# Tony-Tseng/deep-rawburst-sr

Hardware: AMD Instinct MI355X
Metric: bursts/sec 14x48x48 RAW->4x (SyntheticBurstVal shape), DBSR forward (higher is better)
Workload: dtype fp16; 1 GPU; configs[1]: SyntheticBurstVal 14-frame 48x48 -> 384x384 (sr x8 of RAW, x4 of full-res), batch 8 per GPU, full PWC-Net + warp + fusion + decoder; global_batch=8, frames=14, height=48, width=48, out_size=384, parallelism=dp1 (independent bursts per rank), hip_graph=True, fusion_weights_written=True

## Files before the change

### deep-rawburst-sr_amd/csrc/conv128.hip

```cpp
#include "conv_core.hpp"

#include <algorithm>

namespace dbsr {

namespace ks128 {
constexpr int HW = TW + 2, HH = TH + 2, HPX = HW * HH;
constexpr int CPX = 184;
constexpr int NCH = 4;
constexpr int CH_U4 = CPX * 4;
constexpr int PIECES = NCH * CPX / 16;
constexpr int BUF_U4 = NCH * CH_U4;
constexpr int NW = 8;
constexpr int PER = (PIECES + NW - 1) / NW;
#ifndef DBSR_KS_NB
#define DBSR_KS_NB 2
#endif
#ifndef DBSR_KS_ABL
#define DBSR_KS_ABL 0
#endif
#ifndef DBSR_KS_RING
#define DBSR_KS_RING 3
#endif
constexpr int NB = DBSR_KS_NB;
constexpr int RING = DBSR_KS_RING;
constexpr int HALF = TH / 2;
constexpr int XCH_U4 = NW * HALF * 2 * 64;
constexpr int LDS_U4 = 2 * BUF_U4 + XCH_U4;
static_assert(LDS_U4 * 16 + 128 * 4 <= 160 * 1024, "ks128 LDS");
static_assert(CPX % 8 == 0 && CPX >= HPX && (NCH * CPX) % 16 == 0, "chunk images");
static_assert(HALF % NB == 0, "batches");
}

template <typename T, int EPI>
__global__ __launch_bounds__(512, 1) void conv3x3_ks128_kernel(ConvK k, int tiles_x, int tiles_y, int ntiles) {
    using namespace ks128;
    DBSR_OWN_SIMDS();
    __shared__ __attribute__((aligned(16))) u32x4_t lds[LDS_U4 + 32];
    u32x4_t* xch = lds + 2 * BUF_U4;
    float* lbias = (float*)(lds + LDS_U4);
    const int lane = threadIdx.x & 63, wave = __builtin_amdgcn_readfirstlane(threadIdx.x >> 6);
    const int kh = wave >> 2, q = wave & 3;
    const int H = k.in_h, W = k.in_w;
    constexpr bool RT = EPI == 0 || EPI == 5, has_gate = EPI == 5;
    const bool has_res = EPI == 2 || (RT && k.r != nullptr);
    auto act1 = [&](float v) {
        if constexpr (EPI == 1) return fmaxf(v, 0.f);
        else if constexpr (RT) return apply_act(v, k.act);
        else return v;
    };
    auto act2 = [&](float v) {
        if constexpr (EPI == 2) return fmaxf(v, 0.f);
        else if constexpr (RT) return apply_act(v, k.post_act);
        else return v;
    };

    Frag<T> w[2][9][2];
    {
        const char* wsrc = (const char*)k.w_pipe;
#pragma unroll
        for (int c = 0; c < 2; ++c)
#pragma unroll
            for (int tap = 0; tap < 9; ++tap)
#pragma unroll
                for (int h = 0; h < 2; ++h)
                    w[c][tap][h].load((const T*)(wsrc + (((2 * q + h) * NCH + 2 * kh + c) * 9 + tap) * 1024 + lane * 16));
    }
    if (threadIdx.x < 128) lbias[threadIdx.x] = k.bias ? k.bias[threadIdx.x] : 0.f;
    struct Tile { const T* xf; long long y_off, r_off, g_off; int y0, x0; };
    auto decode = [&](int i) {
        const int t = rb_tile(i, blockIdx.x, gridDim.x, ntiles);
        const int tx = t % tiles_x, r = t / tiles_x, ty = r % tiles_y, f = r / tiles_y;
        Tile tl;
        tl.y0 = ty * TH; tl.x0 = tx * TW;
        tl.xf = (const T*)k.x + map_frame(k.xm, f) * k.x_is;
        const long long pix = (long long)tl.y0 * k.out_w + tl.x0;
        tl.y_off = map_frame(k.ym, f) * k.y_is + k.y_c0 + pix * k.y_ld;
        tl.r_off = has_res ? map_frame(k.rm, f) * k.r_is + k.r_c0 + pix * k.r_ld : 0;
        tl.g_off = has_gate ? map_frame(k.gm, f) * k.g_is + k.g_c0 + pix * k.g_ld : 0;
        return tl;
    };
    const int my_tiles = ntiles / (int)gridDim.x + ((int)blockIdx.x < ntiles % (int)gridDim.x ? 1 : 0);

    const int pix_b = k.x_ld * (int)sizeof(T);
    const unsigned frame_bytes = (unsigned)((long long)H * W * pix_b);
    const unsigned lds0 = (unsigned)(unsigned long long)(__attribute__((address_space(3))) u32x4_t*)lds;
    int h_rc[PER], h_off[PER];
#pragma unroll
    for (int it = 0; it < PER; ++it) {
        const int item = min(wave + NW * it, PIECES - 1);
        const int qq = item * 16 + (lane >> 2), c = qq / CPX, p = qq - c * CPX, ph = lane & 3;
        const int gg = 2 * ((ph & 1) ^ ((p >> 2) & 1)) + (ph >> 1);
        const int r = p / HW, cc = p - r * HW;
        h_rc[it] = p < HPX ? (r << 16) | cc : 0x7fff7fff;
        h_off[it] = (r * W + cc) * pix_b + c * 64 + gg * 16;
    }
    auto dma = [&](int it, const Tile& tl, int buf) {
        const int item = min(wave + NW * it, PIECES - 1);
        const int hy = tl.y0 - 1 + (h_rc[it] >> 16), hx = tl.x0 - 1 + (h_rc[it] & 0xffff);
        const bool ok = (unsigned)hy < (unsigned)H && (unsigned)hx < (unsigned)W;
        const int base = ((tl.y0 - 1) * W + (tl.x0 - 1)) * pix_b;
        lds_dma16(tl.xf, frame_bytes, ok ? base + h_off[it] : BUF_OOB, 0,
                  lds0 + (unsigned)((buf * BUF_U4 + item * 64) * 16));
    };

    auto taps = [&](int buf, auto j0_, f32x4_t (&acc)[NB][2], auto&& hook) {
        constexpr int J0 = decltype(j0_)::value, NS = 18;
        if constexpr ((DBSR_KS_ABL & 1) != 0) {
            for (int j = 0; j < NB; ++j) acc[j][0] = acc[j][1] = f32x4_t{(float)(J0 + j + buf), 0.f, 0.f, 0.f};
            StaticFor<0, NS>::run([&](auto s_) { hook(decltype(s_)::value); });
            return;
        }
        const int g = lane >> 4, col = lane & 15;
        const unsigned base = lds0 + (unsigned)((buf * BUF_U4 + kh * 2 * CH_U4) * 16);
        unsigned ba[8];
#pragma unroll
        for (int rho = 0; rho < 8; ++rho) ba[rho] = base + 16u * (4 * col + halo_phys(col + rho, g));
        Frag<T> bq[NB][RING];
        constexpr int AH = RING - 1;
        auto rd = [&](auto j_, auto st_) {
            constexpr int j = decltype(j_)::value, st = decltype(st_)::value;
            constexpr int c = st / 9, tap = st % 9, imm = (J0 + j + tap / 3) * HW + tap % 3;
            const unsigned a = ba[imm & 7];
            bf16x8_t v;
            asm volatile("ds_read_b128 %0, %1 offset:%2" : "=v"(v) : "v"(a), "i"(16 * (c * CH_U4 + 4 * imm)));
            bq[j][st % RING].v = v;
        };
        StaticFor<0, AH>::run([&](auto s0_) {
            StaticFor<0, NB>::run([&](auto j_) { rd(j_, s0_); });
        });
        StaticFor<0, NS>::run([&](auto s_) {
            constexpr int st = decltype(s_)::value, c = st / 9, tap = st % 9;
            const f32x4_t z = {0.f, 0.f, 0.f, 0.f};
            StaticFor<0, NB>::run([&](auto j_) {
                constexpr int j = decltype(j_)::value;
                constexpr int mid = (AH - 1 < NS - 1 - st) ? AH - 1 : NS - 1 - st;
                constexpr int newer = (NB - 1 - j) + NB * mid + (st + AH < NS ? j : 0);
                bf16x8_t v = bq[j][st % RING].v;
                asm volatile("s_waitcnt lgkmcnt(%1)" : "+v"(v) : "i"(newer));
                bq[j][st % RING].v = v;
                acc[j][0] = mma(w[c][tap][0], bq[j][st % RING], st == 0 ? z : acc[j][0]);
                acc[j][1] = mma(w[c][tap][1], bq[j][st % RING], st == 0 ? z : acc[j][1]);
                if constexpr (st + AH < NS) rd(j_, std::integral_constant<int, st + AH>{});
            });
            hook(st);
        });
    };

    Tile cur = decode(0);
    if (my_tiles > 0) {
#pragma unroll
        for (int it = 0; it < PER; ++it) dma(it, cur, 0);
    }
    const int own0 = HALF * kh;
    for (int ti = 0; ti < my_tiles; ++ti) {
        if (ti == 0) vm_drain();
        else DBSR_VM_WAIT(HALF);
        __syncthreads();
        const bool more = ti + 1 < my_tiles;
        const Tile nxt = more ? decode(ti + 1) : cur;
        const int buf = ti & 1;
        int ln = lane;
        asm volatile("" : "+v"(ln));
        const int g = ln >> 4, col = ln & 15;
        StaticFor<0, HALF / NB>::run([&](auto b_) {
            constexpr int b = decltype(b_)::value;
            f32x4_t acc[NB][2];
            auto hook = [&](int st) {
                if constexpr (b == 0 && (DBSR_KS_ABL & 2) == 0) {
                    if (more) {
#pragma unroll
                        for (int it = 0; it < PER; ++it)
                            if (st == 2 * it + 1) dma(it, nxt, buf ^ 1);
                    }
                }
            };
            if (kh == 0) taps(buf, std::integral_constant<int, HALF + NB * b>{}, acc, hook);
            else taps(buf, std::integral_constant<int, NB * b>{}, acc, hook);
#pragma unroll
            for (int j = 0; j < NB; ++j)
#pragma unroll
                for (int h = 0; h < 2; ++h)
                    if constexpr ((DBSR_KS_ABL & 4) == 0)
                        xch[((wave * HALF + NB * b + j) * 2 + h) * 64 + ln] = __builtin_bit_cast(u32x4_t, acc[j][h]);
                    else if (acc[j][h][0] == 12345.f) xch[ln] = u32x4_t{0u, 0u, 0u, 0u};
        });
        u32x4_t resv[HALF];
        auto load_res = [&]() {
#pragma unroll
            for (int j = 0; j < HALF; ++j)
                resv[j] = *(const u32x4_t*)((const T*)k.r + cur.r_off + ((long long)(own0 + j) * k.out_w + col) * k.r_ld +
                                            32 * q + 8 * g);
        };
        if (!RT && has_res) load_res();
        f32x4_t mine[HALF][2];
        StaticFor<0, HALF / NB>::run([&](auto b_) {
            constexpr int b = decltype(b_)::value;
            f32x4_t acc[NB][2];
            auto hook = [&](int) {};
            if (kh == 0) taps(buf, std::integral_constant<int, NB * b>{}, acc, hook);
            else taps(buf, std::integral_constant<int, HALF + NB * b>{}, acc, hook);
#pragma unroll
            for (int j = 0; j < NB; ++j) {
                mine[NB * b + j][0] = acc[j][0];
                mine[NB * b + j][1] = acc[j][1];
            }
        });
        if constexpr ((DBSR_KS_ABL & 4) == 0) dma_barrier();
        const int partner = wave ^ 4;
        const float4 b0 = *(const float4*)(lbias + 32 * q + 8 * g), b1 = *(const float4*)(lbias + 32 * q + 8 * g + 4);
        const float bv[8] = {b0.x, b0.y, b0.z, b0.w, b1.x, b1.y, b1.z, b1.w};
        if (RT && has_res) load_res();
        u32x4_t gatev[has_gate ? HALF : 1];
        if constexpr (has_gate) {
#pragma unroll
            for (int j = 0; j < HALF; ++j)
                gatev[j] = *(const u32x4_t*)((const T*)k.gt + cur.g_off + ((long long)(own0 + j) * k.out_w + col) * k.g_ld +
                                             32 * q + 8 * g);
        }
#pragma unroll
        for (int j = 0; j < HALF; ++j) {
            f32x4_t o0 = {0.f, 0.f, 0.f, 0.f}, o1 = o0;
            if constexpr ((DBSR_KS_ABL & 4) == 0) {
                o0 = __builtin_bit_cast(f32x4_t, xch[((partner * HALF + j) * 2 + 0) * 64 + ln]);
                o1 = __builtin_bit_cast(f32x4_t, xch[((partner * HALF + j) * 2 + 1) * 64 + ln]);
            }
            float v[8];
#pragma unroll
            for (int r = 0; r < 4; ++r) {
                v[r] = act1((mine[j][0][r] + o0[r]) + bv[r]);
                v[4 + r] = act1((mine[j][1][r] + o1[r]) + bv[4 + r]);
            }
            if (has_res) {
#pragma unroll
                for (int e = 0; e < 4; ++e) {
                    v[2 * e] = act2(v[2 * e] + H16<T>::lo(resv[j][e]));
                    v[2 * e + 1] = act2(v[2 * e + 1] + H16<T>::hi(resv[j][e]));
                }
            }
            if constexpr (has_gate) {
#pragma unroll
                for (int e = 0; e < 4; ++e) {
                    v[2 * e] = H16<T>::lo(gatev[j][e]) > 0.f ? v[2 * e] : 0.f;
                    v[2 * e + 1] = H16<T>::hi(gatev[j][e]) > 0.f ? v[2 * e + 1] : 0.f;
                }
            }
            u32x4_t o;
#pragma unroll
            for (int e = 0; e < 4; ++e) o[e] = H16<T>::pack(v[2 * e], v[2 * e + 1]);
            *(u32x4_t*)((T*)k.y + cur.y_off + ((long long)(own0 + j) * k.out_w + col) * k.y_ld + 32 * q + 8 * g) = o;
        }
        cur = nxt;
    }
    vm_drain();
}

int ks128_launch(const ConvK& k, int n_frames, bool f16, int epi, int max_blocks, int cus, hipStream_t s) {
    const int tiles_x = k.out_w / ks128::TW, tiles_y = k.out_h / ks128::TH;
    const long long nt = (long long)n_frames * tiles_x * tiles_y;
    DBSR_CHECK_ARG(nt > 0 && nt < (1LL << 31), "conv2d: bad tile count for the K-split 128-channel kernel");
    const int ntiles = (int)nt;
    int grid = max_blocks > 0 ? std::min(max_blocks, cus) : cus;
    grid = std::min(grid, ntiles);
    DBSR_CHECK_ARG(rb_mapping_ok(grid, ntiles), "conv2d: tile mapping out of range (grid %d, %d tiles)", grid, ntiles);
#define DBSR_KS_LAUNCH(TT, E) \
    hipLaunchKernelGGL((conv3x3_ks128_kernel<TT, E>), dim3(grid), dim3(512), 0, s, k, tiles_x, tiles_y, ntiles)
#define DBSR_KS_EPI(TT)                          \
    switch (epi) {                               \
        case 1: DBSR_KS_LAUNCH(TT, 1); break;    \
        case 2: DBSR_KS_LAUNCH(TT, 2); break;    \
        case 3: DBSR_KS_LAUNCH(TT, 3); break;    \
        case 5: DBSR_KS_LAUNCH(TT, 5); break;    \
        default: DBSR_KS_LAUNCH(TT, 0); break;   \
    }
    if (f16) {
        DBSR_KS_EPI(f16_t)
    } else {
        DBSR_KS_EPI(bf16_t)
    }
#undef DBSR_KS_EPI
#undef DBSR_KS_LAUNCH
    DBSR_LAUNCH_CHECK();
    return 0;
}

}
```

### deep-rawburst-sr_amd/csrc/conv_core.hpp

```cpp
#pragma once
#include "common.hpp"

#include <vector>

namespace dbsr {

inline int round_up(int a, int b) { return (a + b - 1) / b * b; }
inline int cin_pad(int cin) { return cin <= 16 ? round_up(cin, 8) : round_up(cin, 32); }


inline bool is16(int dtype) { return dtype == DBSR_BF16 || dtype == DBSR_F16; }
inline int esize(int dtype) { return is16(dtype) ? 2 : 4; }


struct ConvK {
    const void* x; long long x_is; int x_ld; dbsr_frame_map xm; int in_h, in_w;
    const void* w; const float* bias; int Kp, KG, KGp, CG, kw, stride, pad, dil, cout;
    void* y; int y_f32; long long y_is; int y_ld, y_c0; dbsr_frame_map ym; int out_h, out_w;
    int act;
    const void* r; long long r_is; int r_ld, r_c0; dbsr_frame_map rm; int post_act;
    const void* gt; long long g_is; int g_ld, g_c0; dbsr_frame_map gm;
    int out_mode, shuffle, cps;
    int npix;
    int vec_store;
    int ksplit;
    float* ws;
    int cw;
    const void* w_pipe;
    int max_blocks;
    const float* head_w;
    const float* head_b;
    int head_cout;
    int stage_epi;
};

template <typename T> struct Frag;
template <> struct Frag<bf16_t> {
    bf16x8_t v;
    __device__ __forceinline__ void load(const bf16_t* p) { v = *(const bf16x8_t*)p; }
    __device__ __forceinline__ void zero() { v = bf16x8_t{0, 0, 0, 0, 0, 0, 0, 0}; }
};
template <> struct Frag<f16_t> {
    bf16x8_t v;
    __device__ __forceinline__ void load(const f16_t* p) { v = *(const bf16x8_t*)p; }
    __device__ __forceinline__ void zero() { v = bf16x8_t{0, 0, 0, 0, 0, 0, 0, 0}; }
};
template <> struct Frag<float> {
    float4 a, b;
    __device__ __forceinline__ void load(const float* p) { a = *(const float4*)p; b = *(const float4*)(p + 4); }
    __device__ __forceinline__ void load(const bf16_t* p) {
        const u32x4_t q = *(const u32x4_t*)p;
        a = make_float4(__uint_as_float(q[0] << 16), __uint_as_float(q[0] & 0xffff0000u),
                        __uint_as_float(q[1] << 16), __uint_as_float(q[1] & 0xffff0000u));
        b = make_float4(__uint_as_float(q[2] << 16), __uint_as_float(q[2] & 0xffff0000u),
                        __uint_as_float(q[3] << 16), __uint_as_float(q[3] & 0xffff0000u));
    }
    __device__ __forceinline__ void load(const f16_t* p) {
        const u32x4_t q = *(const u32x4_t*)p;
        a = make_float4(H16<f16_t>::lo(q[0]), H16<f16_t>::hi(q[0]), H16<f16_t>::lo(q[1]), H16<f16_t>::hi(q[1]));
        b = make_float4(H16<f16_t>::lo(q[2]), H16<f16_t>::hi(q[2]), H16<f16_t>::lo(q[3]), H16<f16_t>::hi(q[3]));
    }
    __device__ __forceinline__ void zero() { a = make_float4(0, 0, 0, 0); b = a; }
};

__device__ __forceinline__ f32x4_t mma(const Frag<bf16_t>& A, const Frag<bf16_t>& B, f32x4_t c) {
    typedef __attribute__((ext_vector_type(8))) __bf16 bfv;
    return __builtin_amdgcn_mfma_f32_16x16x32_bf16(__builtin_bit_cast(bfv, A.v), __builtin_bit_cast(bfv, B.v), c,
                                                   0, 0, 0);
}
__device__ __forceinline__ f32x4_t mma(const Frag<f16_t>& A, const Frag<f16_t>& B, f32x4_t c) {
    typedef __attribute__((ext_vector_type(8))) _Float16 hv;
    return __builtin_amdgcn_mfma_f32_16x16x32_f16(__builtin_bit_cast(hv, A.v), __builtin_bit_cast(hv, B.v), c, 0, 0, 0);
}
__device__ __forceinline__ f32x4_t mma(const Frag<float>& A, const Frag<float>& B, f32x4_t c) {
    c = __builtin_amdgcn_mfma_f32_16x16x4f32(A.a.x, B.a.x, c, 0, 0, 0);
    c = __builtin_amdgcn_mfma_f32_16x16x4f32(A.a.y, B.a.y, c, 0, 0, 0);
    c = __builtin_amdgcn_mfma_f32_16x16x4f32(A.a.z, B.a.z, c, 0, 0, 0);
    c = __builtin_amdgcn_mfma_f32_16x16x4f32(A.a.w, B.a.w, c, 0, 0, 0);
    c = __builtin_amdgcn_mfma_f32_16x16x4f32(A.b.x, B.b.x, c, 0, 0, 0);
    c = __builtin_amdgcn_mfma_f32_16x16x4f32(A.b.y, B.b.y, c, 0, 0, 0);
    c = __builtin_amdgcn_mfma_f32_16x16x4f32(A.b.z, B.b.z, c, 0, 0, 0);
    c = __builtin_amdgcn_mfma_f32_16x16x4f32(A.b.w, B.b.w, c, 0, 0, 0);
    return c;
}


__device__ __forceinline__ unsigned relu16x2(unsigned v) {
    typedef short s16x2 __attribute__((ext_vector_type(2)));
    return __builtin_bit_cast(unsigned, __builtin_elementwise_max(__builtin_bit_cast(s16x2, v), s16x2{0, 0}));
}
__device__ __forceinline__ int halo_phys(int p, int g) { return 2 * (g & 1) + ((g >> 1) ^ ((p >> 2) & 1)); }


__host__ __device__ __forceinline__ int rb_tile(int i, int b, int nb, int ntiles) {
    if (nb == 256 && (i + 1) * 256 <= ntiles) return i * 256 + (b & 7) * 32 + (b >> 3);
    return i * nb + b;
}


inline bool rb_mapping_ok(int nb, int ntiles) {
    std::vector<unsigned char> seen(ntiles, 0);
    for (int b = 0; b < nb; ++b) {
        const int my = ntiles / nb + (b < ntiles % nb ? 1 : 0);
        for (int i = 0; i < my; ++i) {
            const int t = rb_tile(i, b, nb, ntiles);
            if (t < 0 || t >= ntiles || seen[t]) return false;
            seen[t] = 1;
        }
    }
    return true;
}

int resblock64_launch(const ConvK& k1, const ConvK& k2, int n_frames, bool f16, int max_blocks, int cus,
                      hipStream_t s);
namespace rb64 {
constexpr int TW = 16, TH = 8;
}

int ks128_launch(const ConvK& k, int n_frames, bool f16, int epi, int max_blocks, int cus, hipStream_t s);
namespace ks128 {
constexpr int TW = 16, TH = 8;
}

}
```

Measured before the change: 3271 bursts/s.

## Rewrite 128-channel conv as weight-stationary row-rolling kernel without K-split exchange

Replaces the K-split scheme, where two wave groups each handle half the input chunks and swap partial sums through LDS, with a weight-stationary design. Each wave now owns 16 output channels across all 4 input chunks and keeps those weights in registers. The taps are rolled over halo rows so each LDS read feeds up to three row accumulators, and the epilogue combines output-row pairs with permlane32_swap. This removes the LDS exchange buffer, the extra barrier and the duplicated halo reads, and interleaves the next-tile DMA and residual/gate loads into the MFMA stream on a compile-time checked schedule. The cost is higher register pressure from 36 weight fragments and 8 accumulators per wave, plus a new host-side validation of launch arguments.

```diff
diff --git a/deep-rawburst-sr_amd/csrc/conv128.hip b/deep-rawburst-sr_amd/csrc/conv128.hip
--- a/deep-rawburst-sr_amd/csrc/conv128.hip
+++ b/deep-rawburst-sr_amd/csrc/conv128.hip
@@ -3,44 +3,14 @@
 #include <algorithm>
 
 namespace dbsr {
-
-namespace ks128 {
-constexpr int HW = TW + 2, HH = TH + 2, HPX = HW * HH;
-constexpr int CPX = 184;
-constexpr int NCH = 4;
-constexpr int CH_U4 = CPX * 4;
-constexpr int PIECES = NCH * CPX / 16;
-constexpr int BUF_U4 = NCH * CH_U4;
-constexpr int NW = 8;
-constexpr int PER = (PIECES + NW - 1) / NW;
-#ifndef DBSR_KS_NB
-#define DBSR_KS_NB 2
-#endif
-#ifndef DBSR_KS_ABL
-#define DBSR_KS_ABL 0
-#endif
-#ifndef DBSR_KS_RING
-#define DBSR_KS_RING 3
-#endif
-constexpr int NB = DBSR_KS_NB;
-constexpr int RING = DBSR_KS_RING;
-constexpr int HALF = TH / 2;
-constexpr int XCH_U4 = NW * HALF * 2 * 64;
-constexpr int LDS_U4 = 2 * BUF_U4 + XCH_U4;
-static_assert(LDS_U4 * 16 + 128 * 4 <= 160 * 1024, "ks128 LDS");
-static_assert(CPX % 8 == 0 && CPX >= HPX && (NCH * CPX) % 16 == 0, "chunk images");
-static_assert(HALF % NB == 0, "batches");
-}
 
 template <typename T, int EPI>
 __global__ __launch_bounds__(512, 1) void conv3x3_ks128_kernel(ConvK k, int tiles_x, int tiles_y, int ntiles) {
     using namespace ks128;
     DBSR_OWN_SIMDS();
-    __shared__ __attribute__((aligned(16))) u32x4_t lds[LDS_U4 + 32];
-    u32x4_t* xch = lds + 2 * BUF_U4;
-    float* lbias = (float*)(lds + LDS_U4);
+    __shared__ __attribute__((aligned(16))) u32x4_t lds[LDS_U4];
     const int lane = threadIdx.x & 63, wave = __builtin_amdgcn_readfirstlane(threadIdx.x >> 6);
-    const int kh = wave >> 2, q = wave & 3;
+    const int g = lane >> 4, col = lane & 15;
     const int H = k.in_h, W = k.in_w;
     constexpr bool RT = EPI == 0 || EPI == 5, has_gate = EPI == 5;
     const bool has_res = EPI == 2 || (RT && k.r != nullptr);
@@ -55,18 +25,23 @@
         else return v;
     };
 
-    Frag<T> w[2][9][2];
+    Frag<T> w[NCH][9];
     {
-        const char* wsrc = (const char*)k.w_pipe;
-#pragma unroll
-        for (int c = 0; c < 2; ++c)
-#pragma unroll
-            for (int tap = 0; tap < 9; ++tap)
-#pragma unroll
-                for (int h = 0; h < 2; ++h)
-                    w[c][tap][h].load((const T*)(wsrc + (((2 * q + h) * NCH + 2 * kh + c) * 9 + tap) * 1024 + lane * 16));
-    }
-    if (threadIdx.x < 128) lbias[threadIdx.x] = k.bias ? k.bias[threadIdx.x] : 0.f;
+        const int m = col;
+        const char* wsrc = (const char*)k.w_pipe + (size_t)packed_block(wave, m) * (NCH * 9 * 1024) +
+                           (g * 16 + packed_row(wave, m)) * 16;
+#pragma unroll
+        for (int c = 0; c < NCH; ++c)
+#pragma unroll
+            for (int tap = 0; tap < 9; ++tap) w[c][tap].load((const T*)(wsrc + (c * 9 + tap) * 1024));
+    }
+    const int co4 = lane_cout(wave, 4 * g), co8 = 16 * wave + 8 * (g & 1);
+    float bv[4];
+#pragma unroll
+    for (int r = 0; r < 4; ++r) bv[r] = k.bias ? k.bias[co4 + r] : 0.f;
+    const int prow = (g >> 1) * k.out_w + col;
+    const int yl = prow * k.y_ld + co8, rl = has_res ? prow * k.r_ld + co8 : 0, gl = has_gate ? prow * k.g_ld + co8 : 0;
+
     struct Tile { const T* xf; long long y_off, r_off, g_off; int y0, x0; };
     auto decode = [&](int i) {
         const int t = rb_tile(i, blockIdx.x, gridDim.x, ntiles);
@@ -85,180 +60,141 @@
     const int pix_b = k.x_ld * (int)sizeof(T);
     const unsigned frame_bytes = (unsigned)((long long)H * W * pix_b);
     const unsigned lds0 = (unsigned)(unsigned long long)(__attribute__((address_space(3))) u32x4_t*)lds;
-    int h_rc[PER], h_off[PER];
-#pragma unroll
-    for (int it = 0; it < PER; ++it) {
+    auto piece = [&](int it, int ln, int& rc, int& off) {
         const int item = min(wave + NW * it, PIECES - 1);
-        const int qq = item * 16 + (lane >> 2), c = qq / CPX, p = qq - c * CPX, ph = lane & 3;
-        const int gg = 2 * ((ph & 1) ^ ((p >> 2) & 1)) + (ph >> 1);
+        const int qq = item * 16 + (ln >> 2), c = qq / CPX, p = qq - c * CPX, ph = ln & 3;
+        const int gg = piece_kgroup(p, ph);
         const int r = p / HW, cc = p - r * HW;
-        h_rc[it] = p < HPX ? (r << 16) | cc : 0x7fff7fff;
-        h_off[it] = (r * W + cc) * pix_b + c * 64 + gg * 16;
+        rc = p < HPX ? (r << 16) | cc : 0x7fff7fff;
+        off = (r * W + cc) * pix_b + c * 64 + gg * 16;
+    };
+    int h_rc[RT ? 1 : PER], h_off[RT ? 1 : PER];
+    if constexpr (!RT) {
+#pragma unroll
+        for (int it = 0; it < PER; ++it) piece(it, lane, h_rc[it], h_off[it]);
     }
     auto dma = [&](int it, const Tile& tl, int buf) {
         const int item = min(wave + NW * it, PIECES - 1);
-        const int hy = tl.y0 - 1 + (h_rc[it] >> 16), hx = tl.x0 - 1 + (h_rc[it] & 0xffff);
+        int rc, off;
+        if constexpr (RT) {
+            int ln = lane;
+            asm volatile("" : "+v"(ln));
+            piece(it, ln, rc, off);
+        } else {
+            rc = h_rc[it];
+            off = h_off[it];
+        }
+        const int hy = tl.y0 - 1 + (rc >> 16), hx = tl.x0 - 1 + (rc & 0xffff);
         const bool ok = (unsigned)hy < (unsigned)H && (unsigned)hx < (unsigned)W;
         const int base = ((tl.y0 - 1) * W + (tl.x0 - 1)) * pix_b;
-        lds_dma16(tl.xf, frame_bytes, ok ? base + h_off[it] : BUF_OOB, 0,
-                  lds0 + (unsigned)((buf * BUF_U4 + item * 64) * 16));
-    };
-
-    auto taps = [&](int buf, auto j0_, f32x4_t (&acc)[NB][2], auto&& hook) {
-        constexpr int J0 = decltype(j0_)::value, NS = 18;
-        if constexpr ((DBSR_KS_ABL & 1) != 0) {
-            for (int j = 0; j < NB; ++j) acc[j][0] = acc[j][1] = f32x4_t{(float)(J0 + j + buf), 0.f, 0.f, 0.f};
-            StaticFor<0, NS>::run([&](auto s_) { hook(decltype(s_)::value); });
-            return;
-        }
-        const int g = lane >> 4, col = lane & 15;
-        const unsigned base = lds0 + (unsigned)((buf * BUF_U4 + kh * 2 * CH_U4) * 16);
-        unsigned ba[8];
-#pragma unroll
-        for (int rho = 0; rho < 8; ++rho) ba[rho] = base + 16u * (4 * col + halo_phys(col + rho, g));
-        Frag<T> bq[NB][RING];
-        constexpr int AH = RING - 1;
-        auto rd = [&](auto j_, auto st_) {
-            constexpr int j = decltype(j_)::value, st = decltype(st_)::value;
-            constexpr int c = st / 9, tap = st % 9, imm = (J0 + j + tap / 3) * HW + tap % 3;
-            const unsigned a = ba[imm & 7];
-            bf16x8_t v;
-            asm volatile("ds_read_b128 %0, %1 offset:%2" : "=v"(v) : "v"(a), "i"(16 * (c * CH_U4 + 4 * imm)));
-            bq[j][st % RING].v = v;
-        };
-        StaticFor<0, AH>::run([&](auto s0_) {
-            StaticFor<0, NB>::run([&](auto j_) { rd(j_, s0_); });
-        });
-        StaticFor<0, NS>::run([&](auto s_) {
-            constexpr int st = decltype(s_)::value, c = st / 9, tap = st % 9;
-            const f32x4_t z = {0.f, 0.f, 0.f, 0.f};
-            StaticFor<0, NB>::run([&](auto j_) {
-                constexpr int j = decltype(j_)::value;
-                constexpr int mid = (AH - 1 < NS - 1 - st) ? AH - 1 : NS - 1 - st;
-                constexpr int newer = (NB - 1 - j) + NB * mid + (st + AH < NS ? j : 0);
-                bf16x8_t v = bq[j][st % RING].v;
-                asm volatile("s_waitcnt lgkmcnt(%1)" : "+v"(v) : "i"(newer));
-                bq[j][st % RING].v = v;
-                acc[j][0] = mma(w[c][tap][0], bq[j][st % RING], st == 0 ? z : acc[j][0]);
-                acc[j][1] = mma(w[c][tap][1], bq[j][st % RING], st == 0 ? z : acc[j][1]);
-                if constexpr (st + AH < NS) rd(j_, std::integral_constant<int, st + AH>{});
-            });
-            hook(st);
-        });
-    };
+        lds_dma16(tl.xf, frame_bytes, ok ? base + off : BUF_OOB, 0, lds0 + (unsigned)((buf * BUF_U4 + item * 64) * 16));
+    };
+    unsigned ba[8];
+#pragma unroll
+    for (int rho = 0; rho < 8; ++rho) ba[rho] = lds0 + 16u * (4 * col + frag_slot(col + rho, g));
 
     Tile cur = decode(0);
     if (my_tiles > 0) {
 #pragma unroll
         for (int it = 0; it < PER; ++it) dma(it, cur, 0);
     }
-    const int own0 = HALF * kh;
+    vm_drain();
+    const long long y_pair = 2LL * k.out_w * k.y_ld, r_pair = 2LL * k.out_w * k.r_ld, g_pair = 2LL * k.out_w * k.g_ld;
     for (int ti = 0; ti < my_tiles; ++ti) {
-        if (ti == 0) vm_drain();
-        else DBSR_VM_WAIT(HALF);
+        DBSR_VM_WAIT(TH / 2);
         __syncthreads();
         const bool more = ti + 1 < my_tiles;
         const Tile nxt = more ? decode(ti + 1) : cur;
         const int buf = ti & 1;
-        int ln = lane;
-        asm volatile("" : "+v"(ln));
-        const int g = ln >> 4, col = ln & 15;
-        StaticFor<0, HALF / NB>::run([&](auto b_) {
-            constexpr int b = decltype(b_)::value;
-            f32x4_t acc[NB][2];
-            auto hook = [&](int st) {
-                if constexpr (b == 0 && (DBSR_KS_ABL & 2) == 0) {
-                    if (more) {
-#pragma unroll
-                        for (int it = 0; it < PER; ++it)
-                            if (st == 2 * it + 1) dma(it, nxt, buf ^ 1);
-                    }
-                }
-            };
-            if (kh == 0) taps(buf, std::integral_constant<int, HALF + NB * b>{}, acc, hook);
-            else taps(buf, std::integral_constant<int, NB * b>{}, acc, hook);
-#pragma unroll
-            for (int j = 0; j < NB; ++j)
-#pragma unroll
-                for (int h = 0; h < 2; ++h)
-                    if constexpr ((DBSR_KS_ABL & 4) == 0)
-                        xch[((wave * HALF + NB * b + j) * 2 + h) * 64 + ln] = __builtin_bit_cast(u32x4_t, acc[j][h]);
-                    else if (acc[j][h][0] == 12345.f) xch[ln] = u32x4_t{0u, 0u, 0u, 0u};
-        });
-        u32x4_t resv[HALF];
-        auto load_res = [&]() {
-#pragma unroll
-            for (int j = 0; j < HALF; ++j)
-                resv[j] = *(const u32x4_t*)((const T*)k.r + cur.r_off + ((long long)(own0 + j) * k.out_w + col) * k.r_ld +
-                                            32 * q + 8 * g);
+        f32x4_t acc[TH];
+        u32x4_t resv[TH / 2], gatev[has_gate ? TH / 2 : 1];
+        Frag<T> bq[AHEAD];
+        auto rd = [&](auto n_) {
+            constexpr int n = decltype(n_)::value, c = read_chunk(n), imm = read_pix(n);
+            const unsigned a = ba[imm & 7];
+            bf16x8_t v;
+            asm volatile("ds_read_b128 %0, %1 offset:%2" : "=v"(v) : "v"(a), "i"(16 * (c * CH_U4 + 4 * imm)));
+            bq[n % AHEAD].v = v;
         };
-        if (!RT && has_res) load_res();
-        f32x4_t mine[HALF][2];
-        StaticFor<0, HALF / NB>::run([&](auto b_) {
-            constexpr int b = decltype(b_)::value;
-            f32x4_t acc[NB][2];
-            auto hook = [&](int) {};
-            if (kh == 0) taps(buf, std::integral_constant<int, NB * b>{}, acc, hook);
-            else taps(buf, std::integral_constant<int, HALF + NB * b>{}, acc, hook);
-#pragma unroll
-            for (int j = 0; j < NB; ++j) {
-                mine[NB * b + j][0] = acc[j][0];
-                mine[NB * b + j][1] = acc[j][1];
-            }
-        });
-        if constexpr ((DBSR_KS_ABL & 4) == 0) dma_barrier();
-        const int partner = wave ^ 4;
-        const float4 b0 = *(const float4*)(lbias + 32 * q + 8 * g), b1 = *(const float4*)(lbias + 32 * q + 8 * g + 4);
-        const float bv[8] = {b0.x, b0.y, b0.z, b0.w, b1.x, b1.y, b1.z, b1.w};
-        if (RT && has_res) load_res();
-        u32x4_t gatev[has_gate ? HALF : 1];
-        if constexpr (has_gate) {
-#pragma unroll
-            for (int j = 0; j < HALF; ++j)
-                gatev[j] = *(const u32x4_t*)((const T*)k.gt + cur.g_off + ((long long)(own0 + j) * k.out_w + col) * k.g_ld +
-                                             32 * q + 8 * g);
-        }
-#pragma unroll
-        for (int j = 0; j < HALF; ++j) {
-            f32x4_t o0 = {0.f, 0.f, 0.f, 0.f}, o1 = o0;
-            if constexpr ((DBSR_KS_ABL & 4) == 0) {
-                o0 = __builtin_bit_cast(f32x4_t, xch[((partner * HALF + j) * 2 + 0) * 64 + ln]);
-                o1 = __builtin_bit_cast(f32x4_t, xch[((partner * HALF + j) * 2 + 1) * 64 + ln]);
-            }
+        auto epilogue = [&](auto pr_) {
+            constexpr int pr = decltype(pr_)::value;
+            if (has_res) asm volatile("" : "+v"(resv[pr]));
+            if constexpr (has_gate) asm volatile("" : "+v"(gatev[pr]));
             float v[8];
 #pragma unroll
             for (int r = 0; r < 4; ++r) {
-                v[r] = act1((mine[j][0][r] + o0[r]) + bv[r]);
-                v[4 + r] = act1((mine[j][1][r] + o1[r]) + bv[4 + r]);
+                const float a0 = act1(acc[2 * pr][r] + bv[r]), a1 = act1(acc[2 * pr + 1][r] + bv[r]);
+                const auto s = __builtin_amdgcn_permlane32_swap(__float_as_uint(a0), __float_as_uint(a1), false, false);
+                v[r] = __uint_as_float(s[0]);
+                v[4 + r] = __uint_as_float(s[1]);
             }
             if (has_res) {
 #pragma unroll
                 for (int e = 0; e < 4; ++e) {
-                    v[2 * e] = act2(v[2 * e] + H16<T>::lo(resv[j][e]));
-                    v[2 * e + 1] = act2(v[2 * e + 1] + H16<T>::hi(resv[j][e]));
+                    v[2 * e] = act2(v[2 * e] + H16<T>::lo(resv[pr][e]));
+                    v[2 * e + 1] = act2(v[2 * e + 1] + H16<T>::hi(resv[pr][e]));
                 }
             }
             if constexpr (has_gate) {
 #pragma unroll
                 for (int e = 0; e < 4; ++e) {
-                    v[2 * e] = H16<T>::lo(gatev[j][e]) > 0.f ? v[2 * e] : 0.f;
-                    v[2 * e + 1] = H16<T>::hi(gatev[j][e]) > 0.f ? v[2 * e + 1] : 0.f;
+                    v[2 * e] = H16<T>::lo(gatev[pr][e]) > 0.f ? v[2 * e] : 0.f;
+                    v[2 * e + 1] = H16<T>::hi(gatev[pr][e]) > 0.f ? v[2 * e + 1] : 0.f;
                 }
             }
             u32x4_t o;
 #pragma unroll
             for (int e = 0; e < 4; ++e) o[e] = H16<T>::pack(v[2 * e], v[2 * e + 1]);
-            *(u32x4_t*)((T*)k.y + cur.y_off + ((long long)(own0 + j) * k.out_w + col) * k.y_ld + 32 * q + 8 * g) = o;
-        }
+            *(u32x4_t*)((T*)k.y + cur.y_off + pr * y_pair + yl) = o;
+        };
+
+        StaticFor<0, AHEAD>::run([&](auto n_) { rd(n_); });
+        StaticFor<0, READS>::run([&](auto n_) {
+            constexpr int n = decltype(n_)::value, c = read_chunk(n);
+            constexpr int newer = AHEAD - 1 < READS - 1 - n ? AHEAD - 1 : READS - 1 - n;
+            bf16x8_t v = bq[n % AHEAD].v;
+            asm volatile("s_waitcnt lgkmcnt(%1)" : "+v"(v) : "i"(newer));
+            Frag<T> b;
+            b.v = v;
+            StaticFor<0, 3>::run([&](auto ky_) {
+                constexpr int ky = decltype(ky_)::value;
+                if constexpr (feeds(n, ky)) {
+                    constexpr int y = read_row(n) - ky, tap = 3 * ky + read_kx(n);
+                    const f32x4_t z = {0.f, 0.f, 0.f, 0.f};
+                    acc[y] = mma(w[c][tap], b, kstep(n, ky) == 0 ? z : acc[y]);
+                }
+            });
+            if constexpr (n + AHEAD < READS) rd(std::integral_constant<int, n + AHEAD>{});
+            StaticFor<0, PER>::run([&](auto it_) {
+                constexpr int it = decltype(it_)::value;
+                if constexpr (n == dma_at(it)) {
+                    if (more) dma(it, nxt, buf ^ 1);
+                }
+            });
+            StaticFor<0, TH / 2>::run([&](auto pr_) {
+                constexpr int pr = decltype(pr_)::value;
+                if constexpr (n == res_at(pr, RT)) {
+                    if (has_res) resv[pr] = *(const u32x4_t*)((const T*)k.r + cur.r_off + pr * r_pair + rl);
+                }
+                if constexpr (has_gate && n == gate_at(pr))
+                    gatev[pr] = *(const u32x4_t*)((const T*)k.gt + cur.g_off + pr * g_pair + gl);
+                if constexpr (n == pair_done(pr)) epilogue(pr_);
+            });
+        });
         cur = nxt;
+#pragma unroll
+        for (int rho = 0; rho < 8; ++rho) ba[rho] += buf ? (unsigned)(-BUF_U4 * 16) : (unsigned)(BUF_U4 * 16);
     }
     vm_drain();
 }
 
 int ks128_launch(const ConvK& k, int n_frames, bool f16, int epi, int max_blocks, int cus, hipStream_t s) {
+    const char* why = ks128::launch_error(k.out_h, k.out_w, k.in_h, k.in_w, n_frames, (long long)k.x_ld * 2, k.y_ld,
+                                          k.y_c0, k.r != nullptr, k.r_ld, k.r_c0, k.gt != nullptr, k.g_ld, k.g_c0);
+    DBSR_CHECK_ARG(why == nullptr, "conv2d: the 128-channel weight-stationary kernel cannot run this: %s", why);
     const int tiles_x = k.out_w / ks128::TW, tiles_y = k.out_h / ks128::TH;
     const long long nt = (long long)n_frames * tiles_x * tiles_y;
-    DBSR_CHECK_ARG(nt > 0 && nt < (1LL << 31), "conv2d: bad tile count for the K-split 128-channel kernel");
+    DBSR_CHECK_ARG(nt > 0 && nt < (1LL << 31), "conv2d: bad tile count for the 128-channel weight-stationary kernel");
     const int ntiles = (int)nt;
     int grid = max_blocks > 0 ? std::min(max_blocks, cus) : cus;
     grid = std::min(grid, ntiles);
diff --git a/deep-rawburst-sr_amd/csrc/conv_core.hpp b/deep-rawburst-sr_amd/csrc/conv_core.hpp
--- a/deep-rawburst-sr_amd/csrc/conv_core.hpp
+++ b/deep-rawburst-sr_amd/csrc/conv_core.hpp
@@ -1,5 +1,6 @@
 #pragma once
 #include "common.hpp"
+#include "ks128_sched.hpp"
 
 #include <vector>
 
@@ -118,8 +119,5 @@
 }
 
 int ks128_launch(const ConvK& k, int n_frames, bool f16, int epi, int max_blocks, int cus, hipStream_t s);
-namespace ks128 {
-constexpr int TW = 16, TH = 8;
-}
 
 }
diff --git a/deep-rawburst-sr_amd/csrc/ks128_sched.hpp b/deep-rawburst-sr_amd/csrc/ks128_sched.hpp
--- /dev/null
+++ b/deep-rawburst-sr_amd/csrc/ks128_sched.hpp
@@ -0,0 +1,117 @@
+#pragma once
+
+namespace dbsr {
+namespace ks128 {
+
+constexpr int TW = 16, TH = 8;
+constexpr int HW = TW + 2, HH = TH + 2, HPX = HW * HH;
+constexpr int CPX = 184;
+constexpr int NCH = 4;
+constexpr int CH_U4 = CPX * 4;
+constexpr int PIECES = NCH * CPX / 16;
+constexpr int BUF_U4 = NCH * CH_U4;
+constexpr int NBUF = 2;
+constexpr int NW = 8;
+constexpr int PER = (PIECES + NW - 1) / NW;
+constexpr int LDS_U4 = NBUF * BUF_U4;
+static_assert(LDS_U4 * 16 <= 160 * 1024, "ks128 LDS");
+static_assert(CPX % 8 == 0 && CPX >= HPX && (NCH * CPX) % 16 == 0, "chunk images");
+
+constexpr int frag_slot(int p, int g) { return 2 * (g & 1) + ((g >> 1) ^ ((p >> 2) & 1)); }
+constexpr int piece_kgroup(int p, int ph) { return 2 * ((ph & 1) ^ ((p >> 2) & 1)) + (ph >> 1); }
+constexpr bool swizzle_ok() {
+    for (int p = 0; p < CPX; ++p)
+        for (int g = 0; g < 4; ++g)
+            if (frag_slot(p, g) < 0 || frag_slot(p, g) > 3 || piece_kgroup(p, frag_slot(p, g)) != g) return false;
+    return true;
+}
+static_assert(swizzle_ok(), "ks128 halo swizzle");
+
+constexpr int RPC = HH * 3;
+constexpr int READS = NCH * RPC;
+constexpr int MFMAS = NCH * 9 * TH;
+constexpr int AHEAD = 4;
+constexpr int read_chunk(int n) { return n / RPC; }
+constexpr int read_row(int n) { return n % RPC / 3; }
+constexpr int read_kx(int n) { return n % 3; }
+constexpr int read_pix(int n) { return read_row(n) * HW + read_kx(n); }
+constexpr bool feeds(int n, int ky) { return read_row(n) - ky >= 0 && read_row(n) - ky < TH; }
+constexpr int kstep(int n, int ky) { return read_chunk(n) * 9 + 3 * ky + read_kx(n); }
+constexpr int pair_done(int pr) { return (NCH - 1) * RPC + (2 * pr + 3) * 3 + 2; }
+constexpr int dma_at(int it) { return 3 + 9 * it; }
+constexpr int res_at(int pr, bool late) { return late ? pair_done(pr) - 12 : 2 * RPC + 2 * pr; }
+constexpr int gate_at(int pr) { return pair_done(pr) - 11; }
+
+constexpr bool schedule_ok() {
+    int next[TH] = {}, total = 0;
+    for (int n = 0; n < READS; ++n) {
+        if (read_pix(n) + TW - 1 >= HPX) return false;
+        for (int ky = 0; ky < 3; ++ky)
+            if (feeds(n, ky)) {
+                const int y = read_row(n) - ky;
+                if (kstep(n, ky) != next[y]) return false;
+                ++next[y];
+                ++total;
+            }
+    }
+    for (int y = 0; y < TH; ++y)
+        if (next[y] != NCH * 9) return false;
+    if (total != MFMAS) return false;
+    for (int pr = 0; pr < TH / 2; ++pr) {
+        if (pair_done(pr) >= READS || (pr > 0 && pair_done(pr) <= pair_done(pr - 1))) return false;
+        for (int y = 2 * pr; y < 2 * pr + 2; ++y)
+            for (int n = pair_done(pr) + 1; n < READS; ++n)
+                for (int ky = 0; ky < 3; ++ky)
+                    if (feeds(n, ky) && read_row(n) - ky == y) return false;
+        for (int late = 0; late < 2; ++late)
+            if (res_at(pr, late != 0) < 0 || res_at(pr, late != 0) >= pair_done(pr)) return false;
+        if (gate_at(pr) < 0 || gate_at(pr) >= pair_done(pr)) return false;
+    }
+    for (int it = 0; it < PER; ++it) {
+        if (dma_at(it) < 0 || dma_at(it) >= pair_done(0) || (it > 0 && dma_at(it) <= dma_at(it - 1))) return false;
+        for (int late = 0; late < 2; ++late)
+            if (dma_at(it) >= res_at(0, late != 0)) return false;
+    }
+    return pair_done(TH / 2 - 1) == READS - 1 && AHEAD >= 1 && AHEAD < RPC;
+}
+static_assert(schedule_ok(), "ks128 row-rolling schedule");
+
+constexpr int lane_cout(int p, int m) { return 16 * p + 8 * ((m >> 2) & 1) + 4 * (m >> 3) + (m & 3); }
+constexpr int packed_block(int p, int m) { return 2 * (p >> 1) + (m >> 3); }
+constexpr int packed_row(int p, int m) { return 4 * (2 * (p & 1) + ((m >> 2) & 1)) + (m & 3); }
+constexpr int packed_cout(int blk, int row) {
+    return 64 * (blk >> 2) + 32 * ((blk & 3) >> 1) + 8 * (row >> 2) + 4 * (blk & 1) + (row & 3);
+}
+constexpr bool gather_ok() {
+    bool seen[128] = {};
+    for (int p = 0; p < NW; ++p)
+        for (int m = 0; m < 16; ++m) {
+            const int co = lane_cout(p, m);
+            if (co < 0 || co >= 128 || seen[co]) return false;
+            seen[co] = true;
+            if (packed_block(p, m) < 0 || packed_block(p, m) >= 8 || packed_row(p, m) < 0 || packed_row(p, m) >= 16)
+                return false;
+            if (packed_cout(packed_block(p, m), packed_row(p, m)) != co) return false;
+        }
+    return true;
+}
+static_assert(gather_ok(), "ks128 cout gather");
+
+inline const char* launch_error(int out_h, int out_w, int in_h, int in_w, long long n_frames, long long x_ld_bytes,
+                                int y_ld, int y_c0, bool has_res, int r_ld, int r_c0, bool has_gate, int g_ld,
+                                int g_c0) {
+    if (out_h <= 0 || out_w <= 0 || out_h % TH || out_w % TW) return "frame not a multiple of the 16 x 8 tile";
+    if (in_h != out_h || in_w != out_w) return "input and output frames differ";
+    if (n_frames <= 0) return "no frames";
+    if (n_frames * (out_h / TH) * (out_w / TW) >= (1LL << 31)) return "tile count past 2^31";
+    if (x_ld_bytes < 256 || (long long)in_h * in_w * x_ld_bytes >= (1LL << 31)) return "frame past 32-bit offsets";
+    const long long ldmax = y_ld > r_ld ? (y_ld > g_ld ? y_ld : g_ld) : (r_ld > g_ld ? r_ld : g_ld);
+    if ((long long)TH * out_w * ldmax + 128 >= (1LL << 31)) return "tile rows past 32-bit offsets";
+    if (y_ld % 8 || y_c0 % 8 || y_ld < 128) return "output not 16-byte aligned";
+    if (has_res && (r_ld % 8 || r_c0 % 8)) return "residual not 16-byte aligned";
+    if (has_gate && (g_ld % 8 || g_c0 % 8)) return "gate not 16-byte aligned";
+    return nullptr;
+}
+
+}
+}
```

New measurement: 3305 bursts/s, median of 6. +1.0%, better.
